# consilience-dev/llm-map-reduce-summarizer

Measured on AMD Instinct MI355X. Metric: chunks/sec (whole node) + end-to-end wall-clock, 10h transcript, Llama-3-8B, higher is better.
Workload: dtype bf16

## Files before the change

llm_map_reduce_summarizer_amd/csrc/kernels/stream_gemm.hip:

```cpp
#include "ar_common.h"

namespace {
enum { EPI_BF16 = 0, EPI_F32_PARTIAL = 1, EPI_SWIGLU = 2, EPI_SWIGLU_SPLIT = 3, EPI_RESID_SPLIT = 4 };
constexpr int SS_PARTS = 8;
constexpr int KBLK = 128;
constexpr int LDS_XTRA = 3 * 1024;
constexpr int LDS_BUDGET = 160 * 1024 - LDS_XTRA;

struct NormArgs {
    const float* ssq;
    int ssq_tiles;
    float inv_k, eps;
    bf16* resid;
    int ldr;
    float* ssp;
    int slab_m;
    mrsum_ar::TPPush tp;
};

template <int N>
__device__ __forceinline__ void wait_vmcnt() {
    static_assert(N >= 0 && N < 64, "vmcnt range");
    __builtin_amdgcn_s_waitcnt((N & 15) | (7 << 4) | (15 << 8) | ((N >> 4) << 14));
}
// ... 528 lines not shown
        epi < EPI_BF16 || epi > EPI_RESID_SPLIT)
        return (int)hipErrorInvalidValue;
    const bool split_epi = epi == EPI_SWIGLU_SPLIT || epi == EPI_RESID_SPLIT;
    if (epi != EPI_F32_PARTIAL && !split_epi && splits != 1) return (int)hipErrorInvalidValue;
    if (split_epi && (!parts || !counters)) return (int)hipErrorInvalidValue;
    if (epi == EPI_RESID_SPLIT && (!resid || !ssp || ldr % 4)) return (int)hipErrorInvalidValue;
    if (ssq && (ssq_tiles <= 0 || ssq_tiles % (4 * SS_PARTS))) return (int)hipErrorInvalidValue;
    if (!tp_push_ok(ar, epi, M, N)) return (int)hipErrorInvalidValue;
    NormArgs e;
    e.ssq = ssq; e.ssq_tiles = ssq_tiles; e.inv_k = 1.f / (float)K; e.eps = eps;
    e.resid = (bf16*)resid; e.ldr = ldr; e.ssp = ssp; e.slab_m = 0;
    e.tp = mrsum_ar::tp_push_of((const mrsum_ar::ArHandle*)ar);
    const int kper = K / splits;
    const int mt = (M + 15) / 16;
    dim3 grid(N / (16 * wpb), splits), block(64 * wpb);
    auto X = (const bf16*)x;
    auto Wp = (const unsigned char*)W;
    auto P = (float*)parts;
    const bool xr = M == 1 && kper <= XR_MAX_K && kper % 512 == 0;
#define L8(MT_, EPI_, WPB_)                                                                                      \
    do {                                                                                                         \
        if (MT_ == 1 && xr)                                                                                      \
            stream_fp8_kernel<1, EPI_, WPB_, true><<<grid, block, 0, s>>>(X, ldx, Wp, wscale, K, M, out, ldo, kper, P, \
                                                                          counters, e);                          \
        else                                                                                                     \
            stream_fp8_kernel<MT_, EPI_, WPB_, false><<<grid, block, 0, s>>>(X, ldx, Wp, wscale, K, M, out, ldo,  \
                                                                             kper, P, counters, e);              \
    } while (0)
#define BY_WPB8(MT_, EPI_)                          \
    switch (wpb) {                                  \
        case 4: L8(MT_, EPI_, 4); break;            \
        case 5: L8(MT_, EPI_, 5); break;            \
        case 6: L8(MT_, EPI_, 6); break;            \
        case 7: L8(MT_, EPI_, 7); break;            \
        default: L8(MT_, EPI_, 8); break;           \
    }
#define BY_EPI8(MT_)                                                      \
    if (epi == EPI_BF16) { BY_WPB8(MT_, EPI_BF16) }                       \
    else if (epi == EPI_F32_PARTIAL) { BY_WPB8(MT_, EPI_F32_PARTIAL) }    \
    else if (epi == EPI_SWIGLU) { BY_WPB8(MT_, EPI_SWIGLU) }              \
    else if (epi == EPI_SWIGLU_SPLIT) { BY_WPB8(MT_, EPI_SWIGLU_SPLIT) }  \
    else { BY_WPB8(MT_, EPI_RESID_SPLIT) }
    switch (mt) {
        case 1: BY_EPI8(1); break;
        case 2: BY_EPI8(2); break;
        case 3: BY_EPI8(3); break;
        default: BY_EPI8(4); break;
    }
#undef BY_EPI8
#undef BY_WPB8
#undef L8
    return (int)hipGetLastError();
}
```

llm_map_reduce_summarizer_amd/engine/model.py:

```python

from __future__ import annotations

import hashlib
import math
import os
from dataclasses import dataclass
from typing import Callable, List, Optional

import torch

from .. import ops
from ..ops.reference import Fp8Weight, interleave_gate_up, rope_cos_sin
from ..parallel.dist import AsyncWorks
from .config import ModelConfig


def _seed_for(seed: int, name: str) -> int:
    return int.from_bytes(hashlib.sha1(("%d:%s" % (seed, name)).encode()).digest()[:8], "little") & ((1 << 63) - 1)


def _randn(shape, std: float, seed: int, name: str, device, dtype) -> torch.Tensor:
    g = torch.Generator(device=device)
    g.manual_seed(_seed_for(seed, name))
    t = torch.randn(*shape, generator=g, device=device, dtype=torch.float32 if device.type == "cpu" else dtype)
# ... 54 lines not shown
    def __init__(self, model: "LlamaModel"):
        self.model = model

    def __call__(self, t: torch.Tensor) -> torch.Tensor:
        return t

    def fused_ok(self, rows: int, hidden: int) -> bool:
        return rows <= 64

    def add_rmsnorm(self, parts, residual, ln, eps):
        lp = self.model.local_push()
        if lp.fits_rows(parts):
            return lp.add_rmsnorm(parts, residual, ln, eps)
        return ops.add_rmsnorm_parts(parts, residual, ln, eps)

    def push_ok(self, rows: int, hidden: int) -> bool:
        return _tp_push_enabled() and self.model.local_push().push_ok(rows, hidden)

    def push_handle(self) -> int:
        return self.model.local_push().push_handle()


@dataclass
class LayerWeights:
    ln1: torch.Tensor
    wqkv: torch.Tensor
    wo: torch.Tensor
    ln2: torch.Tensor
    wgu: torch.Tensor
    wdown: torch.Tensor


class LlamaModel:
    def __init__(self, cfg: ModelConfig, device: torch.device, dtype: torch.dtype = torch.bfloat16, seed: int = 0,
                 tp_rank: int = 0, tp_size: int = 1, tp_group=None, weight_dtype: str = "bf16",
                 weights_path: Optional[str] = None):
        if weight_dtype not in ("bf16", "fp8"):
            raise ValueError("weight_dtype must be bf16 or fp8")
        self.weight_dtype = weight_dtype
        if cfg.n_heads % tp_size or cfg.n_kv_heads % tp_size or cfg.ffn % tp_size or cfg.vocab_size % tp_size:
            raise ValueError("%s does not shard over tp=%d" % (cfg.name, tp_size))
        self.cfg, self.device, self.dtype = cfg, torch.device(device), dtype
        self.tp_rank, self.tp_size, self.tp_group = tp_rank, tp_size, tp_group
        self.hq, self.hkv, self.hd = cfg.n_heads // tp_size, cfg.n_kv_heads // tp_size, cfg.head_dim
        self.ffn_local = cfg.ffn // tp_size
        self.vocab_local = cfg.vocab_size // tp_size
        self.scale = 1.0 / math.sqrt(cfg.head_dim)
        if weights_path:
            from .weights import load_hf
            self.layers = [LayerWeights(None, None, None, None, None, None) for _ in range(cfg.n_layers)]
            load_hf(self, weights_path)
        else:
            self._init_weights(seed)
        self.cos_sin = rope_cos_sin(cfg.max_position, cfg.head_dim, cfg.rope_theta, self.device,
                                    scaling=cfg.rope_scaling)
        self.vocab_offset = tp_rank * self.vocab_local
        self.emulate_tp_reduce = False
        self._local_push = None
        self.sequence_parallel = os.environ.get("MRSUM_SP", "1") == "1"
        self.custom_ar = None
        if tp_size > 1 and self.device.type == "cuda" and os.environ.get("MRSUM_CUSTOM_AR", "1") == "1":
            from ..parallel.custom_ar import maybe_custom_all_reduce
            self.custom_ar = maybe_custom_all_reduce(tp_group, shapes=dict(
                hidden=cfg.hidden, k={"o": self.hq * self.hd, "down": self.ffn_local},
                fp8=weight_dtype == "fp8", rows=(1, 16, 64)))

    def _init_weights(self, seed: int) -> None:
        c, dev, dt = self.cfg, self.device, self.dtype
        std = c.init_std
        r, tp, hd = self.tp_rank, self.tp_size, c.head_dim
        ones = lambda: torch.ones(c.hidden, device=dev, dtype=dt)
        self.embed = _randn((c.vocab_size, c.hidden), std, seed, "embed", dev, dt)
        self.layers: List[LayerWeights] = []
        for i in range(c.n_layers):
            wq = _randn((c.n_heads * hd, c.hidden), std, seed, "l%d.wq" % i, dev, dt)
            wk = _randn((c.n_kv_heads * hd, c.hidden), std, seed, "l%d.wk" % i, dev, dt)
            wv = _randn((c.n_kv_heads * hd, c.hidden), std, seed, "l%d.wv" % i, dev, dt)
            qs, ks = self.hq * hd, self.hkv * hd
            wqkv = torch.cat([wq[r * qs:(r + 1) * qs], wk[r * ks:(r + 1) * ks], wv[r * ks:(r + 1) * ks]]).contiguous()
            del wq, wk, wv
            wo = _randn((c.hidden, c.n_heads * hd), std, seed, "l%d.wo" % i, dev, dt)
            wo = wo[:, r * qs:(r + 1) * qs].contiguous()
            f = self.ffn_local
            wg = _randn((c.ffn, c.hidden), std, seed, "l%d.wg" % i, dev, dt)
            wu = _randn((c.ffn, c.hidden), std, seed, "l%d.wu" % i, dev, dt)
            wgu = interleave_gate_up(wg[r * f:(r + 1) * f], wu[r * f:(r + 1) * f]).contiguous()
            del wg, wu
            wd = _randn((c.hidden, c.ffn), std, seed, "l%d.wd" % i, dev, dt)
            wd = wd[:, r * f:(r + 1) * f].contiguous()
            if self.weight_dtype == "fp8":
                wqkv, wo, wgu, wd = (Fp8Weight.quantize(t) for t in (wqkv, wo, wgu, wd))
            self.layers.append(LayerWeights(ones(), wqkv, wo, ones(), wgu, wd))
        self.final_norm = ones()
        lm = _randn((c.vocab_size, c.hidden), std, seed, "lm_head", dev, dt)
        v = self.vocab_local
        self.lm_head = lm[r * v:(r + 1) * v].contiguous()
        del lm
        self._quantize_lm_head()

    def _quantize_lm_head(self) -> None:
        if self.weight_dtype == "fp8" and not isinstance(self.lm_head, Fp8Weight):
            self.lm_head = Fp8Weight.quantize(self.lm_head)

    def weight_bytes(self) -> int:
        def nb(t):
            return t.nbytes() if isinstance(t, Fp8Weight) else t.numel() * t.element_size()
        n = nb(self.embed) + nb(self.lm_head) + nb(self.final_norm)
        for lw in self.layers:
            n += sum(nb(t) for t in (lw.ln1, lw.wqkv, lw.wo, lw.ln2, lw.wgu, lw.wdown))
        return n

    def local_push(self):
        if self._local_push is None:
            from ..parallel.custom_ar import LocalPush
            self._local_push = LocalPush()
        return self._local_push

    def _all_reduce(self, t: torch.Tensor) -> torch.Tensor:
        if self.tp_size > 1:
            if self.custom_ar is not None and self.custom_ar.fits(t):
                self.custom_ar.all_reduce(t)
            else:
                if t.is_cuda and torch.cuda.is_current_stream_capturing():
                    raise RuntimeError("TP all-reduce of %s does not fit the P2P buffers inside a hipGraph "
                                       "capture (lower the decode batch or raise max_bytes)" % (tuple(t.shape),))
                torch.distributed.all_reduce(t, group=self.tp_group)
        return t

    def _all_reduce_async(self, t: torch.Tensor):
        if self.tp_size == 1:
            return None
        if self.custom_ar is not None and self.custom_ar.fits(t):
            self.custom_ar.all_reduce(t)
            return None
        return torch.distributed.all_reduce(t, group=self.tp_group, async_op=True)

    def _sp_backend_ok(self) -> bool:
        return True

    def _sp_host(self) -> bool:
        return self.device.type == "cuda" and torch.distributed.get_backend(self.tp_group) != "nccl"

    def _sp_rows(self, T: int):
        Tp = -(-T // self.tp_size) * self.tp_size
        return Tp, Tp // self.tp_size

    def _sp_shard(self, t: torch.Tensor) -> torch.Tensor:
        T = t.shape[0]
        Tp, Ts = self._sp_rows(T)
        out = torch.zeros(Ts, t.shape[1], dtype=t.dtype, device=t.device)
        lo = self.tp_rank * Ts
        n = max(0, min(T, lo + Ts) - lo)
        if n:
            out[:n] = t[lo:lo + n]
        return out

    def _sp_reduce_scatter_async(self, t: torch.Tensor):
        T = t.shape[0]
        Tp, Ts = self._sp_rows(T)
        if Tp != T:
# ... 191 lines not shown
```

llm_map_reduce_summarizer_amd/ops/hip.py:

```python

from __future__ import annotations

import ctypes
import os
from typing import Optional

import torch

from ._lib import kernels_lib
from .reference import Fp8Weight

_c_int, _c_float, _vp = ctypes.c_int, ctypes.c_float, ctypes.c_void_p

_SIGS = {
    "mrsum_rmsnorm": [_vp, _vp, _vp, _c_int, _c_int, _c_int, _c_int, _c_float, _vp],
    "mrsum_add_rmsnorm": [_vp, _vp, _vp, _vp, _c_int, _c_int, _c_int, _c_int, _c_float, _vp],
    "mrsum_rmsnorm_fp8": [_vp, _vp, _vp, _vp, _vp, _c_int, _c_int, _c_int, _c_int, _c_float, _c_int, _vp],
    "mrsum_rope_kv": [_vp, _c_int, _c_int, _vp, _vp, _vp, _c_int, _vp, _vp, _vp, _c_int, _c_int, _c_int, _c_int,
                      _c_int, _c_int, _vp],
    "mrsum_rope_kv_parts": [_vp, _c_int, _vp, _c_int, _c_int, _vp, _vp, _vp, _c_int, _vp, _vp, _vp, _c_int,
                            _c_int, _c_int, _c_int, _c_int, _vp],
    "mrsum_swiglu": [_vp, _vp, _c_int, _c_int, _vp],
    "mrsum_kv_scatter": [_vp, _c_int, _c_int, _c_int, _vp, _vp, _vp, _vp, _c_int, _vp],
    "mrsum_embed": [_vp, _vp, _vp, _c_int, _c_int, _c_int, _vp],
    "mrsum_attn_prefill": [_vp, _c_int, _vp, _vp, _c_int, _c_int, _vp, _c_int, _c_int, _c_int, _c_int, _c_float, _vp],
    "mrsum_attn_prefill_paged": [_vp, _c_int, _vp, _vp, _c_int, _c_int, _vp, _c_int, _c_int, _c_int, _c_int, _c_float,
                                 _vp,
                                 _vp, _vp, _c_int, _vp, _vp, _c_int, _vp],
    "mrsum_attn_decode_mfma": [_vp, _c_int, _vp, _vp, _vp, _c_int, _vp, _vp, _vp, _vp, _c_int, _c_int, _c_int,
                               _c_int, _c_int, _c_int, _c_int, _c_float, _vp, _c_int, _vp],
    "mrsum_attn_decode_rope": [_vp, _c_int, _vp, _vp, _vp, _vp, _c_int, _vp, _vp, _vp, _vp, _c_int, _c_int,
                               _c_int, _c_int, _c_int, _c_int, _c_int, _c_float, _vp, _c_int, _vp],
    "mrsum_skinny_gemm": [_vp, _c_int, _vp, _c_int, _c_int, _c_int, _vp, _c_int, _c_int, _c_int, _c_int, _vp, _c_int,
                          _c_float, _vp, _c_int, _vp, _vp, _c_int, _vp],
    "mrsum_skinny_resid_capacity_w": [_c_int],
    "mrsum_skinny_lds": [_vp, _c_int, _vp, _c_int, _c_int, _c_int, _vp, _c_int, _c_int, _c_int, _c_int, _vp],
    "mrsum_stream_gemm": [_vp, _c_int, _vp, _c_int, _c_int, _c_int, _vp, _c_int, _c_int, _c_int, _c_int, _vp, _vp,
                          _vp, _c_int, _c_float, _vp, _c_int, _vp, _c_int, _vp, _vp],
    "mrsum_stream_fp8": [_vp, _c_int, _vp, _vp, _c_int, _c_int, _c_int, _vp, _c_int, _c_int, _c_int, _c_int, _vp, _vp,
                         _vp, _c_int, _c_float, _vp, _c_int, _vp, _vp, _vp],
    "mrsum_skinny_fp8": [_vp, _c_int, _vp, _vp, _c_int, _c_int, _c_int, _vp, _c_int, _c_int, _c_int, _c_int, _vp,
                         _c_int, _c_float, _vp, _c_int, _vp, _vp, _c_int, _vp],
    "mrsum_skinny_fp8_resid_capacity": [],
    "mrsum_quant_fp8_rows": [_vp, _c_int, _vp, _vp, _c_int, _c_int, _vp],
    "mrsum_add_rmsnorm_parts": [_vp, _c_int, _vp, _vp, _vp, _c_int, _c_int, _c_int, _c_float, _vp],
    "mrsum_sample_keys": [_vp, _c_int, _c_int, _c_int, _c_int, _vp, _vp, _vp, _vp, _vp],
    "mrsum_sample_finish": [_vp, _vp, _vp, _vp, _vp, _vp, _c_int, _vp, _vp, _c_int, _vp],
    "mrsum_gemm": [_vp, _c_int, _vp, _c_int, _vp, _c_int, _c_int, _c_int, _c_int, _c_int, _c_int, _vp, _vp, _c_int,
                   _c_int, _vp],
    "mrsum_sample": [_vp, _c_int, _c_int, _c_int, _vp, _vp, _vp, _vp, _vp, _vp, _vp, _vp, _vp, _c_int, _vp, _vp,
                     _vp],
    "mrsum_penalize": [_vp, _c_int, _c_int, _c_int, _c_int, _vp, _c_int, _vp, _vp, _vp, _vp, _vp, _vp],
    "mrsum_penalize_scan": [_vp, _c_int, _c_int, _c_int, _c_int, _vp, _c_int, _vp, _vp, _vp, _vp, _vp, _vp],
    "mrsum_constrain": [_vp, _c_int, _c_int, _c_int, _c_int, _vp, _vp, _c_int, _vp, _vp, _vp, _vp, _vp, _vp, _vp],
    "mrsum_sample_finish_stops": [_vp, _vp, _vp, _vp, _vp, _vp, _c_int, _vp, _vp, _vp, _c_int, _vp],
    "mrsum_sample_keys_filtered": [_vp, _c_int, _c_int, _c_int, _vp, _vp, _vp, _vp, _vp, _vp, _vp, _vp, _vp, _vp],
    "mrsum_sample_thresh": [_vp, _c_int, _c_int, _c_int, _vp, _vp, _vp, _vp, _vp, _vp, _vp],
    "mrsum_sample_filtered": [_vp, _c_int, _c_int, _c_int, _vp, _vp, _vp, _vp, _vp, _vp, _vp, _vp, _vp, _vp, _vp,
                              _vp, _vp, _c_int, _vp, _vp, _vp],
}

_fns = {}


def _fn(name: str):
    f = _fns.get(name)
    if f is None:
        lib = kernels_lib()
        f = getattr(lib, name)
        f.argtypes = _SIGS[name]
        f.restype = ctypes.c_int
        _fns[name] = f
    return f


def _stream() -> int:
    return torch.cuda.current_stream().cuda_stream


def _p(t: Optional[torch.Tensor]) -> Optional[int]:
    return None if t is None else t.data_ptr()


DEBUG_SYNC = os.environ.get("MRSUM_DEBUG_SYNC", "0") == "1"


def _check(rc: int, name: str) -> None:
    if rc != 0:
        raise RuntimeError("%s launch failed: hipError %d" % (name, rc))
    if DEBUG_SYNC and not torch.cuda.is_current_stream_capturing():
        try:
            torch.cuda.synchronize()
        except RuntimeError as e:
# ... 709 lines not shown
    N = w.shape[0]
    if M > SKINNY_MAX_M and epi in (EPI_BF16, EPI_F32_PARTIAL, EPI_SWIGLU) and norm is None:
        ch = STREAM_TALL_M
        for r0 in range(0, M, ch):
            r1 = min(M, r0 + ch)
            if r1 - r0 > SKINNY_MAX_M:
                tw = tall_wpb(N, r1 - r0, splits)
                if tw is not None:
                    o = out[:, r0:r1] if epi == EPI_F32_PARTIAL else out[r0:r1]
                    _stream_launch(x[r0:r1], w, o, epi, splits, ldo, tw, None, None, None, None, None,
                                   M if epi == EPI_F32_PARTIAL else 0)
                    continue
            for c0 in range(r0, r1, SKINNY_MAX_M):
                c1 = min(r1, c0 + SKINNY_MAX_M)
                o = out[:, c0:c1] if epi == EPI_F32_PARTIAL else out[c0:c1]
                _stream_launch(x[c0:c1], w, o, epi, splits, ldo, wpb, None, None, None, None, None,
                               M if epi == EPI_F32_PARTIAL else 0)
        return out
    return _stream_launch(x, w, out, epi, splits, ldo, wpb, parts, counters, norm, resid, ssp, 0, ar)


STREAM_TALL_M = 128
_TALL_WPB = {6: (4, 5, 6), 8: (4, 5)}


def tall_wpb(N: int, M: int, splits: int) -> Optional[int]:
    mt = 6 if M <= 96 else 8
    best, key = None, None
    for wpb in _TALL_WPB[mt]:
        if N % (16 * wpb):
            continue
        grid = N // (16 * wpb) * splits
        k = (round(grid / (-(-grid // N_CU) * N_CU), 3), wpb)
        if key is None or k > key:
            best, key = wpb, k
    return best


def _stream_launch(x, w, out, epi, splits, ldo, wpb, parts, counters, norm, resid, ssp, slab_m, ar=None):
    M, K = x.shape
    N = w.shape[0]
    _req(w.is_contiguous() and w.shape[1] == K, "stream_gemm: weight must be [N, K] contiguous")
    tall_ok = M <= 128 and epi in (EPI_BF16, EPI_F32_PARTIAL, EPI_SWIGLU) and norm is None
    _req(1 <= M and (M <= SKINNY_MAX_M or tall_ok) and K % 128 == 0 and 4 <= wpb <= 8 and N % (16 * wpb) == 0
         and (K // 128) % splits == 0, "stream_gemm: unsupported shape M=%d N=%d K=%d S=%d wpb=%d"
         % (M, N, K, splits, wpb))
    if epi in (EPI_SWIGLU_SPLIT, EPI_RESID_SPLIT):
        _req(parts is not None and parts.shape == (splits, M, N) and parts.dtype == torch.float32
             and counters is not None and counters.numel() >= N // (16 * wpb), "stream_gemm: split-K scratch")
    if epi == EPI_RESID_SPLIT:
        _req(ssp.shape[1] == N // (16 * wpb), "stream_gemm: ssp tiles")
    sq, tiles, eps = _norm_args(x, norm)
    rp, ldr, sp = _resid_args(x, N, epi, resid, ssp)
    _check(_fn("mrsum_stream_gemm")(_p(x), x.stride(0), _p(w), N, K, M, _p(out), ldo, epi, splits, wpb, _p(parts),
                                    _p(counters), sq, tiles, eps, rp, ldr, sp, slab_m, ar, _stream()), "stream_gemm")
    return out


def linear_takes_norm(M: int, N: int, K: int) -> bool:
    return 1 <= M <= SKINNY_MAX_M and K % 128 == 0 and stream_config(N, K, splits=1) is not None


def linear(x: torch.Tensor, w: torch.Tensor, out: Optional[torch.Tensor] = None, norm=None) -> torch.Tensor:
    M, K = x.shape
    N = w.shape[0]
    _req(norm is None or linear_takes_norm(M, N, K), "linear: a deferred norm needs a stream-GEMM shape")
    tall = (SKINNY_MAX_M < M <= STREAM_TALL_M and K % 128 == 0 and norm is None
            and stream_config(N, K, splits=1) is not None and tall_wpb(N, M, 1) is not None)
    if (M > SKINNY_MAX_M and not tall) or M == 0 or K % 128:
        return gemm(x, w, out=out)
    if out is None:
        out = torch.empty(M, N, dtype=x.dtype, device=x.device)
    _req(out.is_contiguous() and out.shape == (M, N), "linear: bad out")
    if tall:
        return _stream_gemm(x, w, out, EPI_BF16, 1, N, tall_wpb(N, M, 1))
    cfg = stream_config(N, K, splits=1)
    if cfg is not None:
        return _stream_gemm(x, w, out, EPI_BF16, 1, N, cfg[0], norm=norm)
    nt = 2 if N % 32 == 0 and N >= 16384 else 1
    if N % (16 * nt):
        return gemm(x, w, out=out)
    return _skinny(x, w, out, EPI_BF16, nt, 1, N)


def linear_parts(x: torch.Tensor, w: torch.Tensor, splits: Optional[int] = None,
                 out: Optional[torch.Tensor] = None, nt: int = 1, kernel: str = "skinny", norm=None) -> torch.Tensor:
    M, K = x.shape
    N = w.shape[0]
    if splits is None:
        splits = choose_splits(N, K, nt if kernel == "skinny" else 4)
    if out is None:
        out = torch.empty(splits, M, N, dtype=torch.float32, device=x.device)
    _req(out.is_contiguous() and out.shape == (splits, M, N) and out.dtype == torch.float32, "linear_parts: bad out")
    if kernel == "stream":
        return _stream_gemm(x, w, out, EPI_F32_PARTIAL, splits, N, nt, norm=norm)
    _req(norm is None, "linear_parts: a deferred norm needs the stream kernel")
    if kernel == "lds":
        return _skinny_lds(x, w, out, EPI_F32_PARTIAL, splits, N)
    return _skinny(x, w, out, EPI_F32_PARTIAL, nt, splits, N)


_TILE_COUNTERS = {}


def _tile_counters(device, n: int) -> torch.Tensor:
    key = (str(device), n)
    t = _TILE_COUNTERS.get(key)
    if t is None:
        _req(not torch.cuda.is_current_stream_capturing(), "split-K SwiGLU tickets first used inside a capture")
# ... 53 lines not shown
        STATS["tp_push"] += 1
    if fp8:
        _skinny_fp8(x, w, None, EPI_SKINNY_RESID, 1, 1, 0, resid=residual, ssp=ssp, ar=tp)
    else:
        _skinny(x, w, None, EPI_SKINNY_RESID, 1, 1, 0, resid=residual, ssp=ssp, ar=tp)
    return ssp


def skinny_fp8_resid_capacity() -> int:
    if "fp8" not in _RESID_CAP:
        _RESID_CAP["fp8"] = int(_fn("mrsum_skinny_fp8_resid_capacity")())
    return _RESID_CAP["fp8"]


def linear_swiglu(x: torch.Tensor, w_gu: torch.Tensor, out: Optional[torch.Tensor] = None,
                  kernel: str = "skinny", wpb: int = 4, splits: int = 1, norm=None) -> torch.Tensor:
    M = x.shape[0]
    F2 = w_gu.shape[0]
    _req(norm is None or kernel in ("stream", "stream_split", "skinny"),
         "linear_swiglu: a deferred norm needs the stream or register-streaming kernel")
    if kernel == "gemm" or M > (STREAM_MAX_M_SWIGLU if kernel == "stream" else SKINNY_MAX_M):
        return gemm(x, w_gu, out=out, swiglu=True)
    if out is None:
        out = torch.empty(M, F2 // 2, dtype=x.dtype, device=x.device)
    _req(out.is_contiguous() and out.shape == (M, F2 // 2), "linear_swiglu: bad out")
    if kernel == "stream":
        return _stream_gemm(x, w_gu, out, EPI_SWIGLU, 1, F2 // 2, wpb, norm=norm)
    if kernel == "stream_split":
        return stream_swiglu_split(x, w_gu, out, wpb, splits, norm=norm)
    if kernel == "lds":
        return _skinny_lds(x, w_gu, out, EPI_SWIGLU, 1, F2 // 2)
    return _skinny(x, w_gu, out, EPI_SWIGLU, 1, 1, F2 // 2, norm=norm)


def add_rmsnorm_parts(parts: torch.Tensor, residual: torch.Tensor, w: torch.Tensor, eps: float,
                      out: Optional[torch.Tensor] = None) -> torch.Tensor:
    _req(parts.is_cuda and parts.dtype == torch.float32 and parts.is_contiguous() and parts.dim() == 3,
         "add_rmsnorm_parts: parts must be fp32 [S, T, D]")
    _bf16_cuda(residual, w)
    S, T, D = parts.shape
    _req(residual.shape == (T, D) and residual.is_contiguous() and w.numel() == D and w.is_contiguous()
         and D % 8 == 0 and D <= 16384, "add_rmsnorm_parts: shapes")
    if out is None:
        out = torch.empty(T, D, dtype=residual.dtype, device=residual.device)
    _bf16_cuda(out)
    _rows_ok(out)
    _req(out.shape == (T, D), "add_rmsnorm_parts: bad out shape")
    _check(_fn("mrsum_add_rmsnorm_parts")(_p(parts), S, _p(residual), _p(w), _p(out), T, D, out.stride(0), eps,
                                          _stream()), "add_rmsnorm_parts")
    return out


N_CU = 256
STATS = {"tp_push": 0}


def stream_config(N: int, K: int, swiglu: bool = False, splits: Optional[int] = None, max_splits: int = 16):
    if K % 128:
        return None
    nkb = K // 128
    best, best_key = None, None
    for wpb in (4, 5, 6, 7, 8):
        if N % (16 * wpb):
            continue
        tiles = N // (16 * wpb)
        cands = [1] if swiglu else ([splits] if splits else range(1, max_splits + 1))
        for S in cands:
            if nkb % S:
                continue
            grid = tiles * S
            eff = grid / (-(-grid // N_CU) * N_CU)
            key = (round(eff, 3), -S, wpb if grid <= 2 * N_CU else -wpb)
            if best_key is None or key > best_key:
                best, best_key = (wpb, S), key
    if best is None or best_key[0] < 0.7:
        return None
    return best


def tp_resid_config(N: int, K: int):
    best, best_key = None, None
    for wpb in (4, 8):
        if N % (16 * wpb) or (N // (16 * wpb)) % 32:
            continue
        tiles = N // (16 * wpb)
        for S in range(1, 17):
            if (K // 128) % S:
                continue
            grid = tiles * S
            eff = grid / (-(-grid // N_CU) * N_CU)
            key = (round(eff, 3), -S, wpb)
            if best_key is None or key > best_key:
                best, best_key = (wpb, S), key
    return best


def swiglu_split_config(N: int, K: int):
    best, best_key = None, None
    for wpb in (4, 7, 8):
        if N % (16 * wpb):
            continue
        tiles = N // (16 * wpb)
        for S in (1, 2, 4, 8, 16):
            if (K // 128) % S or tiles * S > 2 * N_CU:
                continue
            grid = tiles * S
            key = (round(grid / (-(-grid // N_CU) * N_CU), 3), -S, wpb)
# ... 217 lines not shown
```

llm_map_reduce_summarizer_amd/ops/reference.py:

```python

from __future__ import annotations

import math
from typing import Optional

import torch

LOG2E = 1.4426950408889634


def rmsnorm(x: torch.Tensor, w: torch.Tensor, eps: float, out: Optional[torch.Tensor] = None) -> torch.Tensor:
    xf = x.float()
    y = xf * torch.rsqrt(xf.pow(2).mean(-1, keepdim=True) + eps) * w.float()
    y = y.to(x.dtype)
    if out is not None:
        out.copy_(y)
        return out
    return y


def add_rmsnorm(x: torch.Tensor, residual: torch.Tensor, w: torch.Tensor, eps: float,
                out: Optional[torch.Tensor] = None) -> torch.Tensor:
    residual.copy_((x.float() + residual.float()).to(residual.dtype))
    return rmsnorm(residual, w, eps, out)
# ... 109 lines not shown
    kcache[pg, :, sl, :] = r[:, 0].to(kcache.dtype)
    vcache[pg, :, sl, :] = r[:, 1].to(vcache.dtype)


def interleave_gate_up(wg: torch.Tensor, wu: torch.Tensor) -> torch.Tensor:
    f, h = wg.shape
    return torch.stack([wg.reshape(f // 8, 8, h), wu.reshape(f // 8, 8, h)], dim=1).reshape(2 * f, h)


def split_gate_up(gu: torch.Tensor):
    f = gu.shape[-1] // 2
    v = gu.reshape(*gu.shape[:-1], f // 8, 2, 8)
    return v[..., 0, :].reshape(*gu.shape[:-1], f), v[..., 1, :].reshape(*gu.shape[:-1], f)


def swiglu(gu: torch.Tensor, out: Optional[torch.Tensor] = None) -> torch.Tensor:
    g, u = split_gate_up(gu)
    g, u = g.float(), u.float()
    y = (g * torch.sigmoid(g) * u).to(gu.dtype)
    if out is not None:
        out.copy_(y)
        return out
    return y


class Fp8Weight:

    def __init__(self, q: torch.Tensor, scale: torch.Tensor):
        self.q, self.scale = q, scale

    @property
    def shape(self):
        return self.q.shape

    def numel(self) -> int:
        return self.q.numel()

    def nbytes(self) -> int:
        return self.q.numel() + 4 * self.scale.numel()

    def dequant(self, dtype=torch.float32) -> torch.Tensor:
        return (self.q.float() * self.scale.float()[:, None]).to(dtype)

    @staticmethod
    def quantize(w: torch.Tensor) -> "Fp8Weight":
        wf = w.float()
        scale = wf.abs().amax(dim=1).clamp_min(1e-12) / 448.0
        q = (wf / scale[:, None]).clamp(-448.0, 448.0).to(torch.float8_e4m3fn)
        return Fp8Weight(q.contiguous(), scale.contiguous())


def _w(w):
    return w.dequant(torch.bfloat16) if isinstance(w, Fp8Weight) else w


def linear(x: torch.Tensor, w) -> torch.Tensor:
    if isinstance(w, Fp8Weight):
        return (x.float() @ w.dequant().t()).to(x.dtype)
    return torch.nn.functional.linear(x, w)


def linear_parts(x: torch.Tensor, w: torch.Tensor, splits: int = 1) -> torch.Tensor:
    K = x.shape[1]
    ks = K // splits
    wf = w.dequant() if isinstance(w, Fp8Weight) else w.float()
    return torch.stack([x[:, i * ks:(i + 1) * ks].float() @ wf[:, i * ks:(i + 1) * ks].t()
                        for i in range(splits)])


def linear_swiglu(x: torch.Tensor, w_gu) -> torch.Tensor:
    return swiglu(linear(x, w_gu))


def add_rmsnorm_parts(parts: torch.Tensor, residual: torch.Tensor, w: torch.Tensor, eps: float,
                      out: Optional[torch.Tensor] = None) -> torch.Tensor:
    residual.copy_((parts.float().sum(0) + residual.float()).to(residual.dtype))
    return rmsnorm(residual, w, eps, out)


def embed(ids: torch.Tensor, table: torch.Tensor, out: Optional[torch.Tensor] = None) -> torch.Tensor:
    y = table[ids.long().clamp(0, table.shape[0] - 1)]
    if out is not None:
        out.copy_(y)
        return out
    return y


def attn_prefill(qkv: torch.Tensor, cu_seqlens: torch.Tensor, hq: int, hkv: int, d: int, scale: float,
                 out: Optional[torch.Tensor] = None) -> torch.Tensor:
    T = qkv.shape[0]
    if out is None:
        out = torch.empty(T, hq * d, dtype=qkv.dtype, device=qkv.device)
    cu = cu_seqlens.tolist()
    g = hq // hkv
    for i in range(len(cu) - 1):
        s, e = cu[i], cu[i + 1]
        if e <= s:
            continue
        n = e - s
        q = qkv[s:e, : hq * d].view(n, hq, d).float().transpose(0, 1)
        k = qkv[s:e, hq * d: (hq + hkv) * d].view(n, hkv, d).float().transpose(0, 1)
        v = qkv[s:e, (hq + hkv) * d: (hq + 2 * hkv) * d].view(n, hkv, d).float().transpose(0, 1)
        k = k.repeat_interleave(g, dim=0)
        v = v.repeat_interleave(g, dim=0)
        sc = torch.matmul(q, k.transpose(1, 2)) * scale
        mask = torch.ones(n, n, dtype=torch.bool, device=qkv.device).triu(1)
# ... 218 lines not shown
```

Before: 2.173.

## Add lossless 14-bit packed bf16 weight format for skinny streaming GEMMs

Adds a packed weight format that stores each bf16 weight in 14 bits: 8 mantissa bits, a 5-bit exponent code relative to a per-matrix base, and a sign bit. Weights are packed once at model load, and a new streaming GEMM kernel decodes them in LDS before feeding MFMA. The kernel is used for gate_up, down and lm_head at small M. The aim is to cut HBM weight traffic for memory-bound decode GEMMs by about 12.5%. In exchange it adds ALU decode work per tile and extra device memory for the packed copies, and it falls back to the bf16 kernel when any exponent lies outside the 31-value window.

```diff
diff --git a/llm_map_reduce_summarizer_amd/csrc/kernels/stream_gemm.hip b/llm_map_reduce_summarizer_amd/csrc/kernels/stream_gemm.hip
--- a/llm_map_reduce_summarizer_amd/csrc/kernels/stream_gemm.hip
+++ b/llm_map_reduce_summarizer_amd/csrc/kernels/stream_gemm.hip
@@ -604,3 +604,231 @@
 #undef L8
     return (int)hipGetLastError();
 }
+
+namespace {
+constexpr int P14_TILE = 3584, P14_NIB = 2048, P14_TWO = 3072;
+typedef unsigned int u32x2 __attribute__((ext_vector_type(2)));
+
+template <int AUX = 0>
+__device__ __forceinline__ void glds4(const void* g, char* lds) {
+    __builtin_amdgcn_global_load_lds((const __attribute__((address_space(1))) void*)g,
+                                     (__attribute__((address_space(3))) void*)lds, 4, 0, AUX);
+}
+
+template <int Q>
+__device__ __forceinline__ uint32_t p14_hi4(uint32_t q4, uint32_t s2, uint32_t base4) {
+    constexpr int SS = Q == 3 ? 7 : Q;
+    const uint32_t c5 = q4 | ((s2 << Q) & 0x10101010u);
+    const uint32_t nz = (c5 + 0x1f1f1f1fu) & 0x20202020u;
+    const uint32_t on = (nz << 3) - (nz >> 5);
+    return (c5 + (on & base4)) | ((s2 << SS) & 0x80808080u);
+}
+
+template <int PAR>
+__device__ __forceinline__ bf16x8 p14_frag(uint32_t l0, uint32_t l1, uint32_t nb, uint32_t s2, uint32_t base4) {
+    const uint32_t h0 = p14_hi4<2 * PAR>(nb & 0x0f0f0f0fu, s2, base4);
+    const uint32_t h1 = p14_hi4<2 * PAR + 1>((nb >> 4) & 0x0f0f0f0fu, s2, base4);
+    const u32x4 o = {__builtin_amdgcn_perm(h0, l0, 0x05010400u), __builtin_amdgcn_perm(h0, l0, 0x07030602u),
+                     __builtin_amdgcn_perm(h1, l1, 0x05010400u), __builtin_amdgcn_perm(h1, l1, 0x07030602u)};
+    return __builtin_bit_cast(bf16x8, o);
+}
+}
+
+template <int MT, int EPI, int WPB>
+__global__ __launch_bounds__(64 * WPB, 1) void stream_p14_kernel(const bf16* __restrict__ x, int ldx,
+                                                                 const unsigned char* __restrict__ W, int base7,
+                                                                 int K, int M, void* __restrict__ out, int ldo,
+                                                                 int kper, float* __restrict__ parts,
+                                                                 int* __restrict__ counters, const NormArgs e) {
+    constexpr int R = 16 * WPB, BM = 16 * MT;
+    constexpr int WBYTES = WPB * P14_TILE, SLOT = WBYTES + BM * 256;
+    constexpr int D = (LDS_BUDGET / SLOT) < 8 ? (LDS_BUDGET / SLOT) : 8;
+    static_assert(D >= 2, "ring too shallow");
+    constexpr int XP = 2 * BM / 8;
+    constexpr int XI = (XP + WPB - 1) / WPB;
+    constexpr int NI = 5 + XI;
+    static_assert(NI * (D - 2) < 64, "vmcnt range");
+    __shared__ __attribute__((aligned(1024))) char lds[D * SLOT + LDS_XTRA];
+    float* const s_ss = reinterpret_cast<float*>(lds + D * SLOT + 1024);
+
+    const int tid = threadIdx.x, lane = tid & 63, w = tid >> 6;
+    const int n0 = blockIdx.x * R;
+    const int ks = blockIdx.y * kper;
+    const int nkb = kper / KBLK;
+
+    const unsigned char* const wsrc = W + ((size_t)(n0 / 16 + w) * (K / KBLK) + ks / KBLK) * P14_TILE;
+    const int prow = lane >> 3, pslot = lane & 7;
+    const bf16* xsrc[XI];
+    int xdst[XI];
+#pragma unroll
+    for (int i = 0; i < XI; ++i) {
+        const int q = w + WPB * i;
+        const int qq = q < XP ? q : 0;
+        const int row = 8 * (qq >> 1) + prow;
+        xsrc[i] = x + (size_t)min(row, M - 1) * ldx + ks + 8 * (8 * (qq & 1) + (pslot ^ prow));
+        xdst[i] = q < XP ? WBYTES + q * 1024 : -1;
+    }
+#define ISSUE14(slot, kb)                                                                            \
+    {                                                                                                \
+        char* base = lds + (slot) * SLOT;                                                            \
+        char* wb = base + w * P14_TILE;                                                              \
+        const unsigned char* ws = wsrc + (size_t)(kb) * P14_TILE;                                    \
+        glds16<2>(ws + 16 * lane, wb);                                                               \
+        glds16<2>(ws + 1024 + 16 * lane, wb + 1024);                                                 \
+        glds16<2>(ws + P14_NIB + 16 * lane, wb + P14_NIB);                                           \
+        glds4<2>(ws + P14_TWO + 4 * lane, wb + P14_TWO);                                             \
+        glds4<2>(ws + P14_TWO + 256 + 4 * lane, wb + P14_TWO + 256);                                 \
+        _Pragma("unroll") for (int i = 0; i < XI; ++i)                                               \
+            glds16(xsrc[i] + (kb) * KBLK, xdst[i] >= 0 ? base + xdst[i] : lds + D * SLOT);           \
+    }
+
+    f32x4 acc[MT];
+#pragma unroll
+    for (int m = 0; m < MT; ++m) acc[m] = f32x4{0.f, 0.f, 0.f, 0.f};
+
+#pragma unroll
+    for (int s = 0; s < D - 1; ++s) ISSUE14(s, min(s, nkb - 1));
+
+    const uint32_t base4 = (uint32_t)(base7 - 1) * 0x01010101u;
+    const int r = lane & 15, g = lane >> 4;
+    for (int j = 0; j < nkb; ++j) {
+        if (j + D - 2 < nkb) wait_vmcnt<NI * (D - 2)>();
+        else wait_vmcnt<0>();
+        raw_barrier();
+        if (j + D - 1 < nkb) ISSUE14((j + D - 1) % D, j + D - 1);
+        const char* wl = lds + (j % D) * SLOT + w * P14_TILE;
+        const char* xl = lds + (j % D) * SLOT + WBYTES;
+        const u32x4 lo0 = *reinterpret_cast<const u32x4*>(wl + 16 * lane);
+        const u32x4 lo1 = *reinterpret_cast<const u32x4*>(wl + 1024 + 16 * lane);
+        const u32x4 nb = *reinterpret_cast<const u32x4*>(wl + P14_NIB + 16 * lane);
+        const u32x2 s2 = *reinterpret_cast<const u32x2*>(wl + P14_TWO + 8 * lane);
+        bf16x8 av[4];
+        av[0] = p14_frag<0>(lo0[0], lo0[1], nb[0], s2.x, base4);
+        av[1] = p14_frag<1>(lo0[2], lo0[3], nb[1], s2.x, base4);
+        av[2] = p14_frag<0>(lo1[0], lo1[1], nb[2], s2.y, base4);
+        av[3] = p14_frag<1>(lo1[2], lo1[3], nb[3], s2.y, base4);
+#pragma unroll
+        for (int i = 0; i < 4; ++i) {
+#pragma unroll
+            for (int m = 0; m < MT; ++m) {
+                const u32x4 bv = *reinterpret_cast<const u32x4*>(xl + img_off(16 * m + r, 4 * i + g));
+                acc[m] = __builtin_amdgcn_mfma_f32_16x16x32_bf16(av[i], __builtin_bit_cast(bf16x8, bv), acc[m], 0, 0, 0);
+            }
+        }
+    }
+#undef ISSUE14
+
+    stream_epilogue<MT, EPI, WPB>(acc, lds, s_ss, n0, M, out, ldo, parts, counters, e);
+}
+
+MRSUM_API int mrsum_stream_p14(const void* x, int ldx, const void* W, int base7, int N, int K, int M, void* out,
+                               int ldo, int epi, int splits, int wpb, void* parts, int* counters, const float* ssq,
+                               int ssq_tiles, float eps, void* resid, int ldr, float* ssp, void* ar, hipStream_t s) {
+    if (M <= 0) return 0;
+    if (wpb < 4 || wpb > 8 || M > 64 || K % KBLK || N % (16 * wpb) || splits < 1 || (K / KBLK) % splits ||
+        epi < EPI_BF16 || epi > EPI_RESID_SPLIT || base7 < 1 || base7 > 97 || ar)
+        return (int)hipErrorInvalidValue;
+    const bool split_epi = epi == EPI_SWIGLU_SPLIT || epi == EPI_RESID_SPLIT;
+    if (epi != EPI_F32_PARTIAL && !split_epi && splits != 1) return (int)hipErrorInvalidValue;
+    if (split_epi && (!parts || !counters)) return (int)hipErrorInvalidValue;
+    if (epi == EPI_RESID_SPLIT && (!resid || !ssp || ldr % 4)) return (int)hipErrorInvalidValue;
+    if (ssq && (ssq_tiles <= 0 || ssq_tiles % (4 * SS_PARTS))) return (int)hipErrorInvalidValue;
+    NormArgs e;
+    e.ssq = ssq; e.ssq_tiles = ssq_tiles; e.inv_k = 1.f / (float)K; e.eps = eps;
+    e.resid = (bf16*)resid; e.ldr = ldr; e.ssp = ssp; e.slab_m = 0;
+    e.tp = mrsum_ar::tp_push_of(nullptr);
+    const int kper = K / splits;
+    const int mt = (M + 15) / 16;
+    dim3 grid(N / (16 * wpb), splits), block(64 * wpb);
+    auto X = (const bf16*)x;
+    auto Wp = (const unsigned char*)W;
+    auto P = (float*)parts;
+#define L14(MT_, EPI_, WPB_) \
+    stream_p14_kernel<MT_, EPI_, WPB_><<<grid, block, 0, s>>>(X, ldx, Wp, base7, K, M, out, ldo, kper, P, counters, e)
+#define BY_WPB14(MT_, EPI_)                         \
+    switch (wpb) {                                  \
+        case 4: L14(MT_, EPI_, 4); break;           \
+        case 5: L14(MT_, EPI_, 5); break;           \
+        case 6: L14(MT_, EPI_, 6); break;           \
+        case 7: L14(MT_, EPI_, 7); break;           \
+        default: L14(MT_, EPI_, 8); break;          \
+    }
+#define BY_EPI14(MT_)                                                      \
+    if (epi == EPI_BF16) { BY_WPB14(MT_, EPI_BF16) }                       \
+    else if (epi == EPI_F32_PARTIAL) { BY_WPB14(MT_, EPI_F32_PARTIAL) }    \
+    else if (epi == EPI_SWIGLU) { BY_WPB14(MT_, EPI_SWIGLU) }              \
+    else if (epi == EPI_SWIGLU_SPLIT) { BY_WPB14(MT_, EPI_SWIGLU_SPLIT) }  \
+    else { BY_WPB14(MT_, EPI_RESID_SPLIT) }
+    switch (mt) {
+        case 1: BY_EPI14(1); break;
+        case 2: BY_EPI14(2); break;
+        case 3: BY_EPI14(3); break;
+        default: BY_EPI14(4); break;
+    }
+#undef BY_EPI14
+#undef BY_WPB14
+#undef L14
+    return (int)hipGetLastError();
+}
+
+namespace {
+__global__ __launch_bounds__(256) void p14_max_kernel(const uint4* __restrict__ W, size_t n16, int* __restrict__ stats) {
+    uint32_t m = 0;
+    for (size_t i = (size_t)blockIdx.x * blockDim.x + threadIdx.x; i < n16; i += (size_t)gridDim.x * blockDim.x) {
+        const uint4 v = W[i];
+        const uint32_t d[4] = {v.x, v.y, v.z, v.w};
+#pragma unroll
+        for (int c = 0; c < 4; ++c) m = max(m, max((d[c] >> 8) & 0x7fu, (d[c] >> 24) & 0x7fu));
+    }
+#pragma unroll
+    for (int o = 32; o > 0; o >>= 1) m = max(m, (uint32_t)__shfl_xor((int)m, o, 64));
+    if ((threadIdx.x & 63) == 0) atomicMax(stats, (int)m);
+}
+
+__global__ __launch_bounds__(64) void p14_pack_kernel(const bf16* __restrict__ W, int K, unsigned char* __restrict__ P,
+                                                      int* __restrict__ stats) {
+    const int lane = threadIdx.x, r = lane & 15, g = lane >> 4;
+    const int nkb = K / KBLK;
+    const size_t tile = blockIdx.x;
+    const int G = (int)(tile / nkb), kb = (int)(tile % nkb);
+    const int base7 = max(stats[0] - 30, 1);
+    const uint4* src = reinterpret_cast<const uint4*>(W + (size_t)(16 * G + r) * K + (size_t)kb * KBLK + 8 * g);
+    uint32_t lo[8], nb[4], s2[2] = {0u, 0u};
+    int bad = 0;
+#pragma unroll
+    for (int i = 0; i < 4; ++i) {
+        const uint4 v = src[4 * i];
+        const uint32_t d[4] = {v.x, v.y, v.z, v.w};
+        lo[2 * i] = lo[2 * i + 1] = nb[i] = 0u;
+#pragma unroll
+        for (int el = 0; el < 8; ++el) {
+            const uint32_t wv = (d[el >> 1] >> (16 * (el & 1))) & 0xffffu;
+            const int e7 = (wv >> 8) & 0x7f, c = e7 ? e7 - base7 + 1 : 0;
+            bad += e7 && (c < 1 || c > 31);
+            const uint32_t c5 = (uint32_t)c & 31u, sg = wv >> 15;
+            const int b = el & 3, q = 2 * (i & 1) + (el >> 2);
+            lo[2 * i + (el >> 2)] |= (wv & 0xffu) << (8 * b);
+            nb[i] |= (c5 & 15u) << (8 * b + 4 * (el >> 2));
+            s2[i >> 1] |= (c5 >> 4) << (8 * b + 4 - q) | sg << (8 * b + 7 - (q == 3 ? 7 : q));
+        }
+    }
+    unsigned char* t = P + tile * P14_TILE;
+    *reinterpret_cast<uint4*>(t + 16 * lane) = make_uint4(lo[0], lo[1], lo[2], lo[3]);
+    *reinterpret_cast<uint4*>(t + 1024 + 16 * lane) = make_uint4(lo[4], lo[5], lo[6], lo[7]);
+    *reinterpret_cast<uint4*>(t + P14_NIB + 16 * lane) = make_uint4(nb[0], nb[1], nb[2], nb[3]);
+    *reinterpret_cast<uint2*>(t + P14_TWO + 8 * lane) = make_uint2(s2[0], s2[1]);
+    if (bad) atomicAdd(stats + 1, bad);
+}
+}
+
+MRSUM_API int mrsum_p14_pack(const void* W, int N, int K, void* packed, int* stats, hipStream_t s) {
+    if (N <= 0 || K <= 0 || N % 16 || K % KBLK || !W || !packed || !stats) return (int)hipErrorInvalidValue;
+    hipError_t rc = hipMemsetAsync(stats, 0, 2 * sizeof(int), s);
+    if (rc != hipSuccess) return (int)rc;
+    const size_t n16 = (size_t)N * K / 8;
+    const int blocks = (int)((n16 + 255) / 256 < 4096 ? (n16 + 255) / 256 : 4096);
+    p14_max_kernel<<<blocks, 256, 0, s>>>((const uint4*)W, n16, stats);
+    p14_pack_kernel<<<(unsigned)((size_t)(N / 16) * (K / KBLK)), 64, 0, s>>>((const bf16*)W, K, (unsigned char*)packed,
+                                                                              stats);
+    return (int)hipGetLastError();
+}
diff --git a/llm_map_reduce_summarizer_amd/engine/model.py b/llm_map_reduce_summarizer_amd/engine/model.py
--- a/llm_map_reduce_summarizer_amd/engine/model.py
+++ b/llm_map_reduce_summarizer_amd/engine/model.py
@@ -130,6 +130,7 @@
             load_hf(self, weights_path)
         else:
             self._init_weights(seed)
+        self._pack_p14()
         self.cos_sin = rope_cos_sin(cfg.max_position, cfg.head_dim, cfg.rope_theta, self.device,
                                     scaling=cfg.rope_scaling)
         self.vocab_offset = tp_rank * self.vocab_local
@@ -180,10 +181,32 @@
         if self.weight_dtype == "fp8" and not isinstance(self.lm_head, Fp8Weight):
             self.lm_head = Fp8Weight.quantize(self.lm_head)
 
+    def _pack_p14(self) -> None:
+        self.p14 = []
+        if self.weight_dtype != "bf16" or self.tp_size != 1 or self.device.type != "cuda" \
+                or self.dtype != torch.bfloat16:
+            return
+        hip = _hip()
+        if not hip.p14_enabled():
+            return
+        todo = [(self.lm_head, "lm_head")]
+        for lw in self.layers:
+            todo += [(lw.wqkv, "qkv"), (lw.wo, "o"), (lw.wgu, "gate_up"), (lw.wdown, "down")]
+        for w, role in todo:
+            if hip.p14_role_used(role) and w.shape[0] % 16 == 0 and w.shape[1] % 128 == 0:
+                self.p14.append(hip.p14_attach(w, role))
+
+    def __del__(self):
+        try:
+            for pw in getattr(self, "p14", ()):
+                _hip().p14_detach(pw.w)
+        except Exception:
+            pass
+
     def weight_bytes(self) -> int:
         def nb(t):
             return t.nbytes() if isinstance(t, Fp8Weight) else t.numel() * t.element_size()
-        n = nb(self.embed) + nb(self.lm_head) + nb(self.final_norm)
+        n = nb(self.embed) + nb(self.lm_head) + nb(self.final_norm) + sum(pw.nbytes() for pw in self.p14)
         for lw in self.layers:
             n += sum(nb(t) for t in (lw.ln1, lw.wqkv, lw.wo, lw.ln2, lw.wgu, lw.wdown))
         return n
diff --git a/llm_map_reduce_summarizer_amd/ops/hip.py b/llm_map_reduce_summarizer_amd/ops/hip.py
--- a/llm_map_reduce_summarizer_amd/ops/hip.py
+++ b/llm_map_reduce_summarizer_amd/ops/hip.py
@@ -39,6 +39,9 @@
                           _vp, _c_int, _c_float, _vp, _c_int, _vp, _c_int, _vp, _vp],
     "mrsum_stream_fp8": [_vp, _c_int, _vp, _vp, _c_int, _c_int, _c_int, _vp, _c_int, _c_int, _c_int, _c_int, _vp, _vp,
                          _vp, _c_int, _c_float, _vp, _c_int, _vp, _vp, _vp],
+    "mrsum_stream_p14": [_vp, _c_int, _vp, _c_int, _c_int, _c_int, _c_int, _vp, _c_int, _c_int, _c_int, _c_int, _vp,
+                         _vp, _vp, _c_int, _c_float, _vp, _c_int, _vp, _vp, _vp],
+    "mrsum_p14_pack": [_vp, _c_int, _c_int, _vp, _vp, _vp],
     "mrsum_skinny_fp8": [_vp, _c_int, _vp, _vp, _c_int, _c_int, _c_int, _vp, _c_int, _c_int, _c_int, _c_int, _vp,
                          _c_int, _c_float, _vp, _c_int, _vp, _vp, _c_int, _vp],
     "mrsum_skinny_fp8_resid_capacity": [],
@@ -854,9 +857,82 @@
         _req(ssp.shape[1] == N // (16 * wpb), "stream_gemm: ssp tiles")
     sq, tiles, eps = _norm_args(x, norm)
     rp, ldr, sp = _resid_args(x, N, epi, resid, ssp)
+    pw = p14_lookup(w) if _P14 else None
+    if pw is not None and M <= SKINNY_MAX_M and not slab_m and ar is None and p14_takes(pw.role, M):
+        STATS["stream_p14"] += 1
+        _check(_fn("mrsum_stream_p14")(_p(x), x.stride(0), _p(pw.packed), pw.base7, N, K, M, _p(out), ldo, epi, splits,
+                                       wpb, _p(parts), _p(counters), sq, tiles, eps, rp, ldr, sp, None, _stream()),
+               "stream_p14")
+        return out
+    STATS["stream_bf16"] += 1
     _check(_fn("mrsum_stream_gemm")(_p(x), x.stride(0), _p(w), N, K, M, _p(out), ldo, epi, splits, wpb, _p(parts),
                                     _p(counters), sq, tiles, eps, rp, ldr, sp, slab_m, ar, _stream()), "stream_gemm")
     return out
+
+
+P14_ROLES = ("qkv", "o", "gate_up", "down", "lm_head")
+_P14_PLAN = {("gate_up", 1), ("gate_up", 16), ("gate_up", 64), ("lm_head", 1), ("lm_head", 16),
+             ("down", 1), ("down", 16)}
+_P14 = {}
+
+
+class PackedWeight:
+
+    def __init__(self, w: torch.Tensor, packed: Optional[torch.Tensor], base7: int, packable: bool, role: str):
+        self.w, self.packed, self.base7, self.packable, self.role = w, packed, base7, packable, role
+
+    def nbytes(self) -> int:
+        return self.packed.numel() if self.packed is not None else 0
+
+
+def p14_enabled() -> bool:
+    return os.environ.get("MRSUM_P14", P14_DEFAULT) == "1"
+
+
+P14_DEFAULT = "1"
+
+
+def p14_bucket(M: int) -> int:
+    return 1 if M == 1 else 16 if M <= 16 else 64
+
+
+def p14_role_used(role: str) -> bool:
+    return any(r == role for r, _ in _P14_PLAN)
+
+
+def p14_takes(role: str, M: int) -> bool:
+    return p14_enabled() and (role, p14_bucket(M)) in _P14_PLAN
+
+
+def p14_pack(w: torch.Tensor):
+    _bf16_cuda(w)
+    _req(w.dim() == 2 and w.is_contiguous() and w.shape[0] % 16 == 0 and w.shape[1] % 128 == 0,
+         "p14_pack: expected a contiguous bf16 [16 n, 128 k] matrix")
+    N, K = w.shape
+    packed = torch.empty(N * K // 4 * 7, dtype=torch.uint8, device=w.device)
+    stats = torch.zeros(2, dtype=torch.int32, device=w.device)
+    _check(_fn("mrsum_p14_pack")(_p(w), N, K, _p(packed), _p(stats), _stream()), "p14_pack")
+    mx, bad = (int(v) for v in stats.tolist())
+    return packed, max(mx - 30, 1), bad
+
+
+def p14_attach(w: torch.Tensor, role: str) -> PackedWeight:
+    _req(role in P14_ROLES, "p14_attach: unknown role %r" % (role,))
+    packed, base7, bad = p14_pack(w)
+    if bad:
+        print("p14: %s weight %s has %d elements outside the exponent window: bf16 kernel kept"
+              % (role, tuple(w.shape), bad))
+        return PackedWeight(w, None, base7, False, role)
+    pw = _P14[(w.data_ptr(), w.shape[0], w.shape[1])] = PackedWeight(w, packed, base7, True, role)
+    return pw
+
+
+def p14_detach(w: torch.Tensor) -> None:
+    _P14.pop((w.data_ptr(), w.shape[0], w.shape[1]), None)
+
+
+def p14_lookup(w: torch.Tensor) -> Optional[PackedWeight]:
+    return _P14.get((w.data_ptr(), w.shape[0], w.shape[1]))
 
 
 def linear_takes_norm(M: int, N: int, K: int) -> bool:
@@ -1016,7 +1092,7 @@
 
 
 N_CU = 256
-STATS = {"tp_push": 0}
+STATS = {"tp_push": 0, "stream_p14": 0, "stream_bf16": 0}
 
 
 def stream_config(N: int, K: int, swiglu: bool = False, splits: Optional[int] = None, max_splits: int = 16):
diff --git a/llm_map_reduce_summarizer_amd/ops/reference.py b/llm_map_reduce_summarizer_amd/ops/reference.py
--- a/llm_map_reduce_summarizer_amd/ops/reference.py
+++ b/llm_map_reduce_summarizer_amd/ops/reference.py
@@ -185,6 +185,69 @@
 
 def _w(w):
     return w.dequant(torch.bfloat16) if isinstance(w, Fp8Weight) else w
+
+
+P14_TILE = 3584
+P14_WINDOW = 31
+_P14_SIGN_SHIFT = (0, 1, 2, 7)
+
+
+def p14_bits(w: torch.Tensor) -> torch.Tensor:
+    return w.contiguous().view(torch.int16).to(torch.int64) & 0xffff
+
+
+def p14_base7(w: torch.Tensor) -> int:
+    return max(int(((p14_bits(w) >> 8) & 0x7f).max()) - (P14_WINDOW - 1), 1)
+
+
+def _p14_lanes(u: torch.Tensor) -> torch.Tensor:
+    N, K = u.shape
+    t = u.reshape(N // 16, 16, K // 128, 4, 4, 8)
+    return t.permute(0, 2, 4, 1, 3, 5).reshape(-1, 64, 4, 8)
+
+
+def p14_pack_ref(w: torch.Tensor):
+    N, K = w.shape
+    assert w.dtype == torch.bfloat16 and N % 16 == 0 and K % 128 == 0
+    u = _p14_lanes(p14_bits(w))
+    base7 = p14_base7(w)
+    e7 = (u >> 8) & 0x7f
+    c = torch.where(e7 == 0, e7, e7 - base7 + 1)
+    bad = int(((e7 != 0) & ((c < 1) | (c > P14_WINDOW))).sum())
+    c5, sg = c & 31, u >> 15
+    T = u.shape[0]
+    lo = (u & 0xff).reshape(T, 64, 2, 16).permute(0, 2, 1, 3).reshape(T, 2048)
+    q4 = c5 & 15
+    nib = (q4[..., :4] | q4[..., 4:] << 4).reshape(T, 1024)
+    two = torch.zeros(T, 64, 2, dtype=torch.int64, device=u.device)
+    for i in range(4):
+        for e in range(8):
+            b, q = e & 3, 2 * (i & 1) + (e >> 2)
+            two[:, :, i >> 1] |= (c5[:, :, i, e] >> 4) << (8 * b + 4 - q)
+            two[:, :, i >> 1] |= sg[:, :, i, e] << (8 * b + 7 - _P14_SIGN_SHIFT[q])
+    two = torch.stack([(two >> (8 * k)) & 0xff for k in range(4)], dim=-1).reshape(T, 512)
+    return torch.cat([lo, nib, two], dim=1).to(torch.uint8).reshape(-1), base7, bad
+
+
+def p14_unpack_ref(packed: torch.Tensor, base7: int, N: int, K: int) -> torch.Tensor:
+    t = packed.reshape(-1, P14_TILE).to(torch.int64)
+    T = t.shape[0]
+    lo = t[:, :2048].reshape(T, 2, 64, 2, 8).permute(0, 2, 1, 3, 4).reshape(T, 64, 4, 8)
+    nb = t[:, 2048:3072].reshape(T, 64, 4, 4)
+    q4 = torch.cat([nb & 15, nb >> 4], dim=-1)
+    tb = t[:, 3072:].reshape(T, 64, 2, 4)
+    two = sum(tb[..., k] << (8 * k) for k in range(4))
+    hi = torch.zeros_like(lo)
+    for i in range(4):
+        for e in range(8):
+            b, q = e & 3, 2 * (i & 1) + (e >> 2)
+            s = two[:, :, i >> 1]
+            c5 = q4[:, :, i, e] | ((s >> (8 * b + 4 - q)) & 1) << 4
+            e7 = torch.where(c5 == 0, c5, c5 + base7 - 1)
+            hi[:, :, i, e] = ((s >> (8 * b + 7 - _P14_SIGN_SHIFT[q])) & 1) << 7 | e7
+    u = (hi << 8 | lo).reshape(N // 16, K // 128, 4, 16, 4, 8).permute(0, 3, 1, 4, 2, 5).reshape(N, K)
+    u = torch.where(u >= 0x8000, u - 0x10000, u)
+    return u.to(torch.int16).view(torch.bfloat16)
 
 
 def linear(x: torch.Tensor, w) -> torch.Tensor:
```

After: 2.250, median of 6. +3.5%, better.
